# DanielPS555/Radix-sort-Merge-Sort-CUDA---Lab-y-practicos-GPGPU-2023

Hardware: AMD Instinct MI355X
Metric: Mkeys/s sorting uint32, n=2^28, 1 GPU (+ merge-sort at 2/4/8) (higher is better)
Workload: dtype u32; 1 GPU; LSD radix sort (8-bit digits, onesweep), n=2^28 uint32 u32, device-resident (BASELINE config 3); n_per_gpu=268435456, algo=radix, key=u32, dist=u32, parallelism=single GPU

## Files before the change

radix-sort-merge-sort-cuda---lab-y-practicos-gpgpu-2023_amd/csrc/segsort.hip:

```cpp
#include "segsort.h"

#include <algorithm>

#include "devutil.h"
#include "host.h"
#include "seg_kernels.h"

namespace labsort {

namespace {

constexpr int BIN_BLOCK = 1024, BIN_SPT = 4;

__global__ __launch_bounds__(BIN_BLOCK) void k_seg_bin(const uint32_t *__restrict__ off, uint32_t nseg, uint32_t n,
                                                        uint32_t max_len, SegEdges e, uint32_t copy1,
                                                        uint32_t *__restrict__ hdr, uint32_t *__restrict__ lists,
                                                        size_t stride, const Plan *__restrict__ hyplan) {
    __shared__ uint32_t cnt[SEG_CLASSES], base[SEG_CLASSES];
    if (hyplan && hyplan->hybrid == 0u) return;
    const uint32_t tid = threadIdx.x, lane = tid & 63u;
    if (tid < (uint32_t)SEG_CLASSES) cnt[tid] = 0u;
    __syncthreads();
    uint32_t cls[BIN_SPT], pos[BIN_SPT];
    bool bad = false;
#pragma unroll
    for (int j = 0; j < BIN_SPT; ++j) {
        const uint32_t seg = blockIdx.x * (uint32_t)(BIN_BLOCK * BIN_SPT) + (uint32_t)j * BIN_BLOCK + tid;
        uint32_t c = SEG_CLASSES;
        if (seg < nseg) {
            const uint32_t a = off[seg], b = off[seg + 1];
            if (b < a || b > n) {
                bad = true;
            } else {
                const uint32_t len = b - a;
                if (max_len && len > max_len) bad = true;
                if (len > 1u || (len == 1u && copy1)) {
                    c = 0u;
#pragma unroll
                    for (int q = 0; q < SEG_CLASSES - 1; ++q) c += len > e.e[q] ? 1u : 0u;
                }
            }
            if (seg == 0u && a != 0u) bad = true;
            if (seg == nseg - 1u && b != n) bad = true;
        }
        cls[j] = c;
        pos[j] = 0u;
        if (lists) {
#pragma unroll
            for (uint32_t cc = 0; cc < (uint32_t)SEG_CLASSES; ++cc) {
                const uint64_t m = __ballot(c == cc);
                if (m == 0ull) continue;
                const uint32_t leader = (uint32_t)__ffsll((long long)m) - 1u;
                uint32_t wb = 0u;
                if (lane == leader) wb = atomicAdd(&cnt[cc], (uint32_t)__popcll(m));
                wb = __shfl(wb, (int)leader);
                if (c == cc) pos[j] = wb + mbcnt64(m);
            }
        }
    }
    if (bad) atomicOr(hdr, 1u);
    if (!lists) return;
    __syncthreads();
    if (tid < (uint32_t)SEG_CLASSES) base[tid] = cnt[tid] ? atomicAdd(hdr + SEG_HDR_CNT + tid, cnt[tid]) : 0u;
    __syncthreads();
#pragma unroll
    for (int j = 0; j < BIN_SPT; ++j) {
        const uint32_t seg = blockIdx.x * (uint32_t)(BIN_BLOCK * BIN_SPT) + (uint32_t)j * BIN_BLOCK + tid;
        if (cls[j] < (uint32_t)SEG_CLASSES) lists[(size_t)cls[j] * stride + base[cls[j]] + pos[j]] = seg;
    }
}

__global__ __launch_bounds__(256) void k_seg_ids(const uint32_t *__restrict__ off, uint32_t nseg, uint32_t n,
                                                 const uint32_t *__restrict__ idx, uint32_t *__restrict__ ids,
                                                 uint32_t *__restrict__ iota, const uint32_t *__restrict__ hdr) {
    if (ld_agent(hdr) != 0u) return;
    const size_t stride = (size_t)gridDim.x * blockDim.x;
    for (size_t i = (size_t)blockIdx.x * blockDim.x + threadIdx.x; i < n; i += stride) {
        if (iota) iota[i] = (uint32_t)i;
        if (!ids) continue;
        uint32_t p = idx ? idx[i] : (uint32_t)i;
        if (p >= n) p = n - 1u;
        uint32_t lo = 1u, hi = nseg;
        while (lo < hi) {
            const uint32_t mid = lo + (hi - lo) / 2u;
            if (off[mid] > p) hi = mid;
            else lo = mid + 1u;
        }
        ids[i] = lo - 1u;
    }
}

__global__ __launch_bounds__(256) void k_seg_gather(const uint32_t *__restrict__ src, const uint32_t *__restrict__ vsrc,
                                                    const uint32_t *__restrict__ perm, uint32_t *__restrict__ out,
                                                    uint32_t *__restrict__ vout, uint32_t n,
                                                    const uint32_t *__restrict__ hdr) {
    if (ld_agent(hdr) != 0u) return;
    const size_t stride = (size_t)gridDim.x * blockDim.x;
    for (size_t i = (size_t)blockIdx.x * blockDim.x + threadIdx.x; i < n; i += stride) {
        uint32_t p = perm ? perm[i] : (uint32_t)i;
        if (p >= n) p = n - 1u;
        out[i] = src[p];
        if (vsrc) vout[i] = vsrc[p];
    }
}

__global__ void k_seg_err_acc(uint32_t *hdr, uint32_t *inner) {
    if (threadIdx.x == 0 && blockIdx.x == 0) {
        if (*inner) hdr[SEG_HDR_DEVERR] = 1u;
        *inner = 0u;
    }
}

unsigned stream_blocks(size_t n) {
    size_t b = (n + 256 * 8 - 1) / (256 * 8);
    return (unsigned)(b < 1 ? 1 : b > 8192 ? 8192 : b);
}

hipError_t launch_seg_sort(int c, const uint32_t *in, uint32_t *out, const uint32_t *vin, uint32_t *vout,
                           const uint32_t *off, const uint32_t *hdr, const uint32_t *list, uint32_t flip,
                           hipStream_t s, const HySel &hy = HySel{}, bool f32 = false) {
    return f32 ? launch_seg_sort_f32(c, in, out, vin, vout, off, hdr, list, flip, s, hy)
               : launch_seg_sort_t<false>(c, in, out, vin, vout, off, hdr, list, flip, s, hy);
}

hipError_t launch_seg_ids(const uint32_t *off, size_t nseg, size_t n, const uint32_t *idx, uint32_t *ids,
                          uint32_t *iota, const uint32_t *hdr, hipStream_t s) {
    k_seg_ids<<<stream_blocks(n), 256, 0, s>>>(off, (uint32_t)nseg, (uint32_t)n, idx, ids, iota, hdr);
    return hipGetLastError();
}

hipError_t launch_seg_gather(const uint32_t *src, const uint32_t *vsrc, const uint32_t *perm, uint32_t *out,
                             uint32_t *vout, size_t n, const uint32_t *hdr, hipStream_t s) {
    k_seg_gather<<<stream_blocks(n), 256, 0, s>>>(src, vsrc, perm, out, vout, (uint32_t)n, hdr);
    return hipGetLastError();
}

hipError_t launch_seg_err_acc(uint32_t *hdr, uint32_t *inner_err, hipStream_t s) {
    k_seg_err_acc<<<1, 64, 0, s>>>(hdr, inner_err);
    return hipGetLastError();
}

}

hipError_t launch_seg_bin(const uint32_t *off, size_t nseg, size_t n, size_t max_len, bool pairs, bool copy1,
                          uint32_t *hdr, uint32_t *lists, size_t stride, hipStream_t s) {
    const unsigned g = (unsigned)((nseg + BIN_BLOCK * BIN_SPT - 1) / (BIN_BLOCK * BIN_SPT));
    (void)pairs;
    const SegEdges e{{(uint32_t)SEG_WAVE_KEYS, (uint32_t)SEG_WAVE2_KEYS, (uint32_t)SEG_WAVE3_KEYS, (uint32_t)SEG_BLOCK_KEYS}};
    k_seg_bin<<<g, BIN_BLOCK, 0, s>>>(off, (uint32_t)nseg, (uint32_t)n, (uint32_t)max_len, e, copy1 ? 1u : 0u, hdr, lists,
                                      stride, nullptr);
    return hipGetLastError();
}

hipError_t launch_seg_lds_classes(size_t max_len, bool pairs, const uint32_t *in, uint32_t *out, const uint32_t *vin,
                                  uint32_t *vout, const uint32_t *off, const uint32_t *hdr, const uint32_t *lists,
                                  size_t stride, uint32_t flip, bool f32, hipStream_t s) {
    size_t edges[SEG_CLASSES];
    labsort_segment_class_edges(pairs ? 1 : 0, edges, SEG_CLASSES);
    int ncls = 1;
    while (ncls < SEG_CLASSES && max_len > edges[ncls - 1]) ++ncls;
    for (int c = 0; c < ncls; ++c) {
        const hipError_t e = launch_seg_sort(c, in, out, vin, vout, off, hdr, lists + (size_t)c * stride, flip, s, HySel{}, f32);
        if (e != hipSuccess) return e;
    }
    return hipSuccess;
}

namespace {
constexpr int FB_BLOCK = 1024;

__global__ __launch_bounds__(FB_BLOCK) void k_fin_bounds(const Plan *__restrict__ plan, Bufs bufs, uint32_t n, uint32_t flip,
                                                         const uint32_t *__restrict__ top14, uint32_t *__restrict__ off) {
    constexpr uint32_t GPB = FB_BLOCK / 4;
    __shared__ uint32_t wsum[FB_BLOCK / WAVE];
    __shared__ uint32_t gstart[GPB + 1];
    if (plan->hybrid == 0u) return;
    const uint32_t *__restrict__ keys = bufs.p[plan->fin_src];
    const uint32_t tid = threadIdx.x, lane = tid & 63u, wid = tid >> 6;
    const uint32_t g0 = blockIdx.x * GPB;
    uint32_t before = 0u;
    for (uint32_t i = tid; i < g0; i += FB_BLOCK) before += top14[i];
    const uint32_t mine = tid < GPB ? top14[g0 + tid] : 0u;
    uint32_t x = mine, tot = before;
#pragma unroll
    for (int o = 1; o < 64; o <<= 1) {
        const uint32_t t = __shfl_up(x, o);
        if (lane >= (uint32_t)o) x += t;
    }
#pragma unroll
    for (int o = 32; o > 0; o >>= 1) tot += __shfl_xor(tot, o);
    if (lane == 63u) wsum[wid] = x;
    __syncthreads();
    uint32_t pre = 0u;
    for (uint32_t w = 0; w < wid && w < GPB / WAVE; ++w) pre += wsum[w];
    __syncthreads();
    if (lane == 0u) wsum[wid] = tot;
    __syncthreads();
    uint32_t base = 0u;
    for (uint32_t w = 0; w < (uint32_t)(FB_BLOCK / WAVE); ++w) base += wsum[w];
    if (tid < GPB) {
        gstart[tid] = base + pre + x - mine;
        if (tid == GPB - 1u) gstart[GPB] = base + pre + x;
    }
    __syncthreads();
    const uint32_t q = blockIdx.x * FB_BLOCK + tid;
    uint32_t lo = min(gstart[tid >> 2], n), hi = min(gstart[(tid >> 2) + 1u], n);
    while (lo < hi) {
        const uint32_t mid = lo + (hi - lo) / 2u;
        if (((keys[mid] ^ flip) >> 16) >= q) hi = mid;
        else lo = mid + 1u;
    }
    off[q] = lo;
    if (q == HY_BUCKETS - 1u) off[HY_BUCKETS] = n;
}
}

hipError_t launch_hybrid_finish(const Plan *plan, Bufs b, size_t n, uint32_t flip, const uint32_t *top14, uint32_t *hdr,
                                uint32_t *off, uint32_t *lists, hipStream_t s) {
    static_assert(HY_BUCKETS % FB_BLOCK == 0 && HY_TOP * 4 == (int)HY_BUCKETS, "four buckets per top-14-bit group");
    const size_t stride = HY_BUCKETS;
    k_fin_bounds<<<HY_BUCKETS / FB_BLOCK, FB_BLOCK, 0, s>>>(plan, b, (uint32_t)n, flip, top14, off);
    hipError_t e = hipGetLastError();
    if (e != hipSuccess) return e;
    const SegEdges ed{{(uint32_t)SEG_WAVE_KEYS, (uint32_t)SEG_WAVE2_KEYS, (uint32_t)SEG_WAVE3_KEYS, (uint32_t)HY_BLOCK_KEYS}};
    k_seg_bin<<<HY_BUCKETS / (BIN_BLOCK * BIN_SPT), BIN_BLOCK, 0, s>>>(off, HY_BUCKETS, (uint32_t)n, HY_MAX_BUCKET, ed, 1u, hdr,
                                                                      lists, stride, plan);
    if ((e = hipGetLastError()) != hipSuccess) return e;
    const HySel hy{plan, {b.p[0], b.p[1], b.p[2]}};
    uint32_t *out = b.p[SEL_OUT];
    const unsigned cus = (unsigned)cu_count();
    for (int c = 0; c < SEG_CLASSES; ++c) {
        const uint32_t *list = lists + (size_t)c * stride;
        if (c == 3) {
            k_seg_block<HY_BLOCK, HY_BLOCK_KPT, false, HY_BLOCK_WPE><<<cus * (unsigned)HY_BLOCK_WPE, HY_BLOCK, 0, s>>>(
                out, out, nullptr, nullptr, off, hdr, list, 3, flip, hy);
            e = hipGetLastError();
        } else {
            e = launch_seg_sort(c, out, out, nullptr, nullptr, off, hdr, list, flip, s, hy);
        }
        if (e != hipSuccess) return e;
    }
    return hipSuccess;
}

size_t seg_inner_bytes(size_t n) {
    const size_t m = n < (size_t)LABSORT_AUTO_PAIRS_MERGE_MAX_KEYS ? n : (size_t)LABSORT_AUTO_PAIRS_MERGE_MAX_KEYS;
    return std::max(labsort_pairs_workspace_bytes(n, LABSORT_ALGO_AUTO), labsort_pairs_workspace_bytes(m, LABSORT_ALGO_MERGE));
}

}

using namespace labsort;

extern "C" {

size_t labsort_segment_tile_keys(void) { return (size_t)SEG_TILE_KEYS; }
size_t labsort_segment_pair_tile_keys(void) { return (size_t)SEG_TILE_PAIRS; }

int labsort_segment_class_edges(int pairs, size_t *edges, int cap) {
    const size_t e[SEG_CLASSES] = {(size_t)SEG_WAVE_KEYS, (size_t)SEG_WAVE2_KEYS, (size_t)SEG_WAVE3_KEYS, (size_t)SEG_BLOCK_KEYS,
                                   pairs ? (size_t)SEG_TILE_PAIRS : (size_t)SEG_TILE_KEYS};
    for (int i = 0; i < SEG_CLASSES && i < cap && edges; ++i) edges[i] = e[i];
    return SEG_CLASSES;
}

namespace {
bool seg_lds_path(size_t max_len, int pairs) {
    return max_len > 0 && max_len <= (pairs ? (size_t)SEG_TILE_PAIRS : (size_t)SEG_TILE_KEYS);
}
struct SegLayout {
    size_t off_lists, list_stride;
    size_t off_a, off_b, off_c, off_inner, inner_bytes;
    size_t total;
};
SegLayout seg_layout(size_t n, size_t nseg, bool lds) {
    SegLayout L{};
    Carver c{SEG_HDR_BYTES};
    if (lds) {
        L.list_stride = align_up(nseg * 4, 256) / 4;
        L.off_lists = c.take((size_t)SEG_CLASSES * L.list_stride * 4);
        L.total = c.o;
    } else {
        L.off_a = c.take(n * 4);
        L.off_b = c.take(n * 4);
        L.off_c = c.take(n * 4);
        L.off_inner = c.o;
        L.inner_bytes = seg_inner_bytes(n);
        L.total = c.o + L.inner_bytes;
    }
    return L;
}

int sort_segments(const uint32_t *ki, const uint32_t *vi, uint32_t *ko, uint32_t *vo, size_t n, const uint32_t *off,
                  size_t nseg, size_t max_len, int key_type, void *d_ws, size_t ws_bytes, void *stream) {
    const bool pairs = vi != nullptr || vo != nullptr;
    if (n == 0) return LABSORT_OK;
    if (!ki || !ko || !off || (pairs && (!vi || !vo))) return LABSORT_ERR_ARG;
    if (!device_key_type_ok(key_type)) return LABSORT_ERR_ARG;
    if (nseg == 0 || n > (size_t)0x7FFFFFFFu || nseg > (size_t)0x7FFFFFFFu) return LABSORT_ERR_ARG;
    if (pairs && !pairs_alias_ok(ki, vi, ko, vo)) return LABSORT_ERR_ARG;
    const bool lds = seg_lds_path(max_len, pairs ? 1 : 0);
    if (!lds && n > RADIX_MAX_N) return LABSORT_ERR_ARG;
    if (!d_ws || ws_bytes < labsort_segments_workspace_bytes(n, nseg, max_len, pairs ? 1 : 0)) return LABSORT_ERR_ARG;
    const SegLayout L = seg_layout(n, nseg, lds);
    const uint32_t flip = flip_of(key_type);
    hipStream_t s = as_stream(stream);
    char *ws = static_cast<char *>(d_ws);
    uint32_t *hdr = reinterpret_cast<uint32_t *>(ws);
    const bool inplace = ki == ko;
    HIP_TRY(launch_zero(hdr, SEG_HDR_BYTES, s));
    if (lds) {
        uint32_t *lists = reinterpret_cast<uint32_t *>(ws + L.off_lists);
        TimingScope ts(LABSORT_K_SEGSORT, s);
        HIP_TRY(launch_seg_bin(off, nseg, n, max_len, pairs, !inplace, hdr, lists, L.list_stride, s));
        HIP_TRY(launch_seg_lds_classes(max_len, pairs, ki, ko, vi, vo, off, hdr, lists, L.list_stride, flip,
                                       key_type == LABSORT_KEY_F32, s));
        return LABSORT_OK;
    }
    uint32_t *A = reinterpret_cast<uint32_t *>(ws + L.off_a), *B = reinterpret_cast<uint32_t *>(ws + L.off_b),
             *C = reinterpret_cast<uint32_t *>(ws + L.off_c);
    char *iws = ws + L.off_inner;
    uint32_t *ierr = reinterpret_cast<uint32_t *>(iws);
    HIP_TRY(launch_zero(ierr, 16, s));
    {
        TimingScope ts(LABSORT_K_SEGSORT, s);
        HIP_TRY(launch_seg_bin(off, nseg, n, max_len, pairs, false, hdr, nullptr, 0, s));
        if (pairs) HIP_TRY(launch_seg_ids(off, nseg, n, nullptr, nullptr, A, hdr, s));
        else HIP_TRY(launch_seg_ids(off, nseg, n, nullptr, A, nullptr, hdr, s));
    }
    int st;
    if ((st = labsort_sort_pairs_device(ki, A, B, C, n, key_type, LABSORT_ALGO_AUTO, iws, L.inner_bytes, stream))) return st;
    HIP_TRY(launch_seg_err_acc(hdr, ierr, s));
    if (pairs) {
        {
            TimingScope ts(LABSORT_K_SEGSORT, s);
            HIP_TRY(launch_seg_ids(off, nseg, n, C, B, nullptr, hdr, s));
        }
        if ((st = labsort_sort_pairs_device(B, C, B, C, n, LABSORT_KEY_U32, LABSORT_ALGO_AUTO, iws, L.inner_bytes, stream)))
            return st;
        HIP_TRY(launch_seg_err_acc(hdr, ierr, s));
        TimingScope ts(LABSORT_K_SEGSORT, s);
        if (inplace) {
            HIP_TRY(launch_seg_gather(ki, vi, C, A, B, n, hdr, s));
            HIP_TRY(launch_seg_gather(A, B, nullptr, ko, vo, n, hdr, s));
        } else {
            HIP_TRY(launch_seg_gather(ki, vi, C, ko, vo, n, hdr, s));
        }
    } else {
        if ((st = labsort_sort_pairs_device(C, B, C, B, n, LABSORT_KEY_U32, LABSORT_ALGO_AUTO, iws, L.inner_bytes, stream)))
            return st;
        HIP_TRY(launch_seg_err_acc(hdr, ierr, s));
        TimingScope ts(LABSORT_K_SEGSORT, s);
        HIP_TRY(launch_seg_gather(B, nullptr, nullptr, ko, nullptr, n, hdr, s));
    }
    return LABSORT_OK;
}
}

size_t labsort_segments_workspace_bytes(size_t n, size_t nseg, size_t max_segment_keys, int pairs) {
    return seg_layout(n, nseg, seg_lds_path(max_segment_keys, pairs)).total;
}

int labsort_sort_segments_device(const void *d_keys_in, void *d_keys_out, size_t n, const uint32_t *d_offsets,
                                 size_t nseg, size_t max_segment_keys, int key_type, void *d_ws, size_t ws_bytes,
                                 void *stream) {
    return sort_segments(static_cast<const uint32_t *>(d_keys_in), nullptr, static_cast<uint32_t *>(d_keys_out), nullptr,
                         n, d_offsets, nseg, max_segment_keys, key_type, d_ws, ws_bytes, stream);
}

int labsort_sort_segments_pairs_device(const void *d_keys_in, const void *d_vals_in, void *d_keys_out, void *d_vals_out,
                                       size_t n, const uint32_t *d_offsets, size_t nseg, size_t max_segment_keys,
                                       int key_type, void *d_ws, size_t ws_bytes, void *stream) {
    if (n == 0) return LABSORT_OK;
    if (!d_vals_in || !d_vals_out) return LABSORT_ERR_ARG;
    return sort_segments(static_cast<const uint32_t *>(d_keys_in), static_cast<const uint32_t *>(d_vals_in),
                         static_cast<uint32_t *>(d_keys_out), static_cast<uint32_t *>(d_vals_out), n, d_offsets, nseg,
                         max_segment_keys, key_type, d_ws, ws_bytes, stream);
}

int labsort_segments_workspace_status(const void *d_ws, void *stream) {
    uint32_t w[2] = {0, 0};
    if (const int st = read_ws_words(d_ws, w, 2, as_stream(stream))) return st;
    return w[0] ? LABSORT_ERR_ARG : w[SEG_HDR_DEVERR] ? LABSORT_ERR_DEVICE : LABSORT_OK;
}

}
```

Baseline: 135,100 Mkeys/s.

## Add dedicated finish kernel for large hybrid buckets with segment prefetch

Replaces the generic segmented block sort used for the largest bucket class in the hybrid radix finish with a specialized kernel. The new kernel runs two 8-bit LDS ranking passes over the low 16 bits, uses a DPP wave scan for the per-wave digit offsets, and prefetches the next segment's keys into registers while the current one is ranked and written. It also drops the flip/key-transform and extra buffer parameters. Register pressure rises from holding two key tiles, which may hurt occupancy. An A/B harness script for timing the finish stage is added.

```diff
diff --git a/harness/finish_ab.py b/harness/finish_ab.py
--- /dev/null
+++ b/harness/finish_ab.py
@@ -0,0 +1,97 @@
+#!/usr/bin/env python3
+import argparse
+import ctypes
+import importlib
+import os
+import statistics
+import sys
+
+import torch
+
+REPO = os.path.dirname(os.path.dirname(os.path.abspath(__file__)))
+sys.path.insert(0, REPO)
+ls = importlib.import_module("radix-sort-merge-sort-cuda---lab-y-practicos-gpgpu-2023_amd")
+
+K_SEGSORT = ls.KCLASS["segsort"]
+ALGO_RADIX = ls.ALGO["radix"]
+
+
+def load(path):
+    if not path:
+        return ls.lib
+    lib = ctypes.CDLL(path)
+    for name in ("labsort_sort_device", "labsort_workspace_bytes", "labsort_workspace_status", "labsort_radix_path",
+                 "labsort_timing_enable", "labsort_timing_read"):
+        f, g = getattr(lib, name), getattr(ls.lib, name)
+        f.argtypes, f.restype = g.argtypes, g.restype
+    return lib
+
+
+def fmt(ts):
+    return f"{statistics.median(ts):7.4f} [{min(ts):7.4f}, {max(ts):7.4f}]"
+
+
+def main():
+    ap = argparse.ArgumentParser()
+    ap.add_argument("--lib", action="append", default=[], help="NAME=PATH; empty PATH: the package's library")
+    ap.add_argument("--sizes", default="1,0.5,1.19", help="comma-separated, in units of 2^28 keys")
+    ap.add_argument("--reps", type=int, default=9)
+    ap.add_argument("--warmup", type=int, default=2)
+    ap.add_argument("--note", default="")
+    ap.add_argument("--out", default="")
+    a = ap.parse_args()
+    if not torch.cuda.is_available():
+        sys.exit("finish_ab: no GPU (no CPU fallback)")
+    out = open(a.out, "a") if a.out else sys.stdout
+    builds = {}
+    for spec in a.lib or ["this="]:
+        name, _, path = spec.partition("=")
+        builds[name] = load(path)
+    st = torch.cuda.current_stream().cuda_stream
+    print(f"# finish A/B{': ' + a.note if a.note else ''}: {torch.cuda.get_device_name(0)}; {a.reps} alternating repetitions "
+          f"after {a.warmup} warm-ups; ms per sort, median [min, max]", file=out)
+    for size in [float(x) for x in a.sizes.split(",")]:
+        n = int(size * (1 << 28))
+        if size == 1.0:
+            os.environ.pop("LABSORT_RADIX_HYBRID", None)
+        else:
+            os.environ["LABSORT_RADIX_HYBRID"] = "2"
+        keys = torch.empty(n, dtype=torch.int32, device="cuda")
+        ls.fill(keys, n, seed=0x5EED0001, dist="u32")
+        res = torch.empty_like(keys)
+        first = None
+        nbytes = max(int(lib.labsort_workspace_bytes(n, ALGO_RADIX)) for lib in builds.values())
+        ws = torch.zeros(nbytes, dtype=torch.uint8, device="cuda")
+        fin = {k: [] for k in builds}
+        tot = {k: [] for k in builds}
+        for rep in range(a.warmup + a.reps):
+            for name, lib in builds.items():
+                lib.labsort_timing_enable(1)
+                e0, e1 = torch.cuda.Event(enable_timing=True), torch.cuda.Event(enable_timing=True)
+                e0.record()
+                rc = lib.labsort_sort_device(keys.data_ptr(), res.data_ptr(), n, 0, ALGO_RADIX, ws.data_ptr(), nbytes, st)
+                e1.record()
+                e1.synchronize()
+                if rc or lib.labsort_workspace_status(ws.data_ptr(), n, ALGO_RADIX, st):
+                    sys.exit(f"finish_ab: {name}: the sort failed")
+                ms, cnt = ctypes.c_double(0.0), ctypes.c_longlong(0)
+                lib.labsort_timing_read(K_SEGSORT, ctypes.byref(ms), ctypes.byref(cnt))
+                lib.labsort_timing_enable(0)
+                if rep == 0:
+                    if int(lib.labsort_radix_path(ws.data_ptr(), n, st)) != 1:
+                        sys.exit(f"finish_ab: {name}: n = {n} did not take the hybrid path")
+                    if first is None:
+                        first = res.clone()
+                    elif not torch.equal(res, first):
+                        sys.exit(f"finish_ab: {name}: result differs from the first build's")
+                if rep >= a.warmup:
+                    fin[name].append(ms.value)
+                    tot[name].append(e0.elapsed_time(e1))
+        for name in builds:
+            print(f"n = {size:g} x 2^28  {name:>8}  finish {fmt(fin[name])}   whole sort (timing hooks on) {fmt(tot[name])}", file=out)
+        out.flush()
+        del keys, res, ws, first
+
+
+if __name__ == "__main__":
+    main()
diff --git a/radix-sort-merge-sort-cuda---lab-y-practicos-gpgpu-2023_amd/csrc/fin_block.h b/radix-sort-merge-sort-cuda---lab-y-practicos-gpgpu-2023_amd/csrc/fin_block.h
--- /dev/null
+++ b/radix-sort-merge-sort-cuda---lab-y-practicos-gpgpu-2023_amd/csrc/fin_block.h
@@ -0,0 +1,204 @@
+#pragma once
+#include "segsort.h"
+
+#include "devutil.h"
+
+namespace labsort {
+
+namespace {
+
+#ifndef LABSORT_FIN_PREFETCH
+#define LABSORT_FIN_PREFETCH 1
+#endif
+
+__device__ __forceinline__ uint32_t wave_incl_scan_dpp(uint32_t x) {
+    x += (uint32_t)__builtin_amdgcn_update_dpp(0, (int)x, 0x111, 0xf, 0xf, false);
+    x += (uint32_t)__builtin_amdgcn_update_dpp(0, (int)x, 0x112, 0xf, 0xf, false);
+    x += (uint32_t)__builtin_amdgcn_update_dpp(0, (int)x, 0x114, 0xf, 0xf, false);
+    x += (uint32_t)__builtin_amdgcn_update_dpp(0, (int)x, 0x118, 0xf, 0xf, false);
+    x += (uint32_t)__builtin_amdgcn_update_dpp(0, (int)x, 0x142, 0xa, 0xf, false);
+    x += (uint32_t)__builtin_amdgcn_update_dpp(0, (int)x, 0x143, 0xc, 0xf, false);
+    return x;
+}
+
+template <int BLOCK, int KPT>
+struct FinSmem {
+    static constexpr int R = 256, W = BLOCK / WAVE, TILE = BLOCK * KPT;
+    static_assert(TILE <= 65536, "16-bit LDS slots");
+    static_assert(W == 4, "the fold holds one counter row per wave in registers");
+    uint32_t keys[TILE];
+    alignas(16) uint32_t cnt[W * R];
+    alignas(16) uint32_t offs[W * R];
+    uint32_t probe[WAVE];
+    uint32_t ordered;
+};
+
+struct FinStripe {
+    size_t sb;
+    uint32_t ws0;
+    uint32_t nf;
+    uint32_t ng;
+    bool tail_ok;
+};
+template <int W, int KPT>
+__device__ __forceinline__ FinStripe fin_stripe(uint32_t b, uint32_t len, uint32_t lane, uint32_t wid) {
+    if (len > (uint32_t)(W * WAVE * KPT)) len = 0u;
+    const uint32_t jn = (len + (uint32_t)(W * WAVE) - 1u) / (uint32_t)(W * WAVE);
+    const uint32_t ws0 = wid * jn * WAVE;
+    const uint32_t rem = ws0 < len ? len - ws0 : 0u;
+    const uint32_t nf = min(jn, rem / WAVE);
+    const uint32_t tail = nf < jn ? rem - nf * WAVE : 0u;
+    return {(size_t)b + ws0, ws0, nf, nf + (tail ? 1u : 0u), lane < tail};
+}
+
+template <int KPT>
+__device__ __forceinline__ void fin_load(const uint32_t *in, const FinStripe &g, uint32_t lane, uint32_t (&k)[KPT]) {
+    const char *pb = reinterpret_cast<const char *>(in + g.sb);
+    const uint32_t lb = lane * 4u;
+    if (g.nf == (uint32_t)KPT) {
+#pragma unroll
+        for (int j = 0; j < KPT; ++j) k[j] = ld_stream<NT_TILE>(reinterpret_cast<const uint32_t *>(pb + (lb + (uint32_t)(j * WAVE * 4))));
+    } else {
+#pragma unroll
+        for (int j = 0; j < KPT; ++j) {
+            k[j] = 0xFFFFFFFFu;
+            if ((uint32_t)j < g.nf || ((uint32_t)j == g.nf && g.tail_ok))
+                k[j] = ld_stream<NT_TILE>(reinterpret_cast<const uint32_t *>(pb + (lb + (uint32_t)(j * WAVE * 4))));
+        }
+    }
+}
+
+template <int BLOCK, int KPT>
+__device__ __forceinline__ void fin_pass(FinSmem<BLOCK, KPT> &sm, const uint32_t (&k)[KPT], uint32_t shift, uint32_t ng,
+                                         bool atomic_rank, uint32_t lane, uint32_t wid) {
+    constexpr int W = FinSmem<BLOCK, KPT>::W, R = FinSmem<BLOCK, KPT>::R;
+    uint32_t *wh = sm.cnt + wid * R;
+    uint32_t *wo = sm.offs + wid * R;
+    uint32_t n0 = ng, n1 = ng;
+    asm volatile("" : "+s"(n0), "+s"(n1));
+    uint32_t z = 0u;
+    asm volatile("" : "+v"(z));
+    *reinterpret_cast<uint4 *>(wh + 4u * lane) = make_uint4(z, z, z, z);
+    uint32_t rank[KPT / 2] = {};
+#pragma unroll
+    for (int j = 0; j < KPT; ++j) {
+        uint32_t r = 0u;
+        if ((uint32_t)j < n0) r = rank8(wh, (k[j] >> shift) & 0xFFu, lane, atomic_rank);
+        set16(rank, j, r);
+    }
+    __syncthreads();
+    {
+        uint4 c[W];
+#pragma unroll
+        for (int w = 0; w < W; ++w) c[w] = *reinterpret_cast<const uint4 *>(sm.cnt + w * R + 4u * lane);
+        uint32_t tot[4] = {0u, 0u, 0u, 0u}, bef[4] = {0u, 0u, 0u, 0u};
+#pragma unroll
+        for (int w = 0; w < W; ++w) {
+            const uint32_t cw[4] = {c[w].x, c[w].y, c[w].z, c[w].w};
+            const bool before = (uint32_t)w < wid;
+#pragma unroll
+            for (int q = 0; q < 4; ++q) {
+                tot[q] += cw[q];
+                bef[q] += before ? cw[q] : 0u;
+            }
+        }
+        const uint32_t s = tot[0] + tot[1] + tot[2] + tot[3];
+        uint32_t run = wave_incl_scan_dpp(s) - s;
+        uint4 o4;
+        o4.x = run + bef[0];
+        run += tot[0];
+        o4.y = run + bef[1];
+        run += tot[1];
+        o4.z = run + bef[2];
+        run += tot[2];
+        o4.w = run + bef[3];
+        *reinterpret_cast<uint4 *>(wo + 4u * lane) = o4;
+    }
+    __builtin_amdgcn_wave_barrier();
+#pragma unroll
+    for (int j = 0; j < KPT; ++j)
+        if ((uint32_t)j < n1) set16(rank, j, wo[(k[j] >> shift) & 0xFFu] + get16(rank, j));
+#pragma unroll
+    for (int j = 0; j < KPT; ++j)
+        if ((uint32_t)j < n1) sm.keys[get16(rank, j)] = k[j];
+    __syncthreads();
+}
+
+template <int BLOCK, int KPT, int WPE>
+__global__ __launch_bounds__(BLOCK, WPE) void k_fin_block(uint32_t *out, const uint32_t *__restrict__ off,
+                                                           const uint32_t *__restrict__ hdr,
+                                                           const uint32_t *__restrict__ list, HySel hy) {
+    using S = FinSmem<BLOCK, KPT>;
+    constexpr int W = S::W;
+    constexpr int CLS = 3;
+    constexpr bool PREFETCH = LABSORT_FIN_PREFETCH != 0;
+    __shared__ S sm;
+    if (hy.plan->hybrid == 0u) return;
+    const uint32_t *in = hy.buf[hy.plan->fin_src];
+    if (ld_agent(hdr) != 0u) return;
+    const uint32_t cnt = hdr[SEG_HDR_CNT + CLS];
+    const uint32_t tid = threadIdx.x, lane = tid & 63u, wid = __builtin_amdgcn_readfirstlane(tid >> 6);
+    if (blockIdx.x >= cnt) return;
+    probe_lane_order(sm.probe, &sm.ordered, lane, wid);
+    __syncthreads();
+    const bool atomic_rank = lane_order_probed(&sm.ordered);
+    uint32_t nb, ne;
+    {
+        const uint32_t seg = __builtin_amdgcn_readfirstlane(list[blockIdx.x]);
+        nb = __builtin_amdgcn_readfirstlane(off[seg]);
+        ne = __builtin_amdgcn_readfirstlane(off[seg + 1]);
+    }
+    uint32_t k[KPT];
+    FinStripe g = fin_stripe<W, KPT>(nb, ne - nb, lane, wid);
+    if constexpr (PREFETCH) fin_load(in, g, lane, k);
+    for (uint32_t it = blockIdx.x; it < cnt; it += gridDim.x) {
+        if constexpr (!PREFETCH) {
+            g = fin_stripe<W, KPT>(nb, ne - nb, lane, wid);
+            fin_load(in, g, lane, k);
+        }
+        const bool more = it + gridDim.x < cnt;
+        if (more) {
+            const uint32_t seg = __builtin_amdgcn_readfirstlane(list[it + gridDim.x]);
+            nb = __builtin_amdgcn_readfirstlane(off[seg]);
+            ne = __builtin_amdgcn_readfirstlane(off[seg + 1]);
+        }
+        fin_pass(sm, k, 0u, g.ng, atomic_rank, lane, wid);
+        {
+            uint32_t n2 = g.ng;
+            asm volatile("" : "+s"(n2));
+#pragma unroll
+            for (int j = 0; j < KPT; ++j)
+                if ((uint32_t)j < n2) k[j] = sm.keys[g.ws0 + (uint32_t)j * WAVE + lane];
+        }
+        fin_pass(sm, k, 8u, g.ng, atomic_rank, lane, wid);
+        FinStripe gn = g;
+        uint32_t kn[PREFETCH ? KPT : 1];
+        if constexpr (PREFETCH) {
+            gn = fin_stripe<W, KPT>(nb, more ? ne - nb : 0u, lane, wid);
+            fin_load(in, gn, lane, kn);
+        }
+        uint32_t nfs = g.nf;
+        asm volatile("" : "+s"(nfs));
+        const uint32_t *sk = sm.keys + g.ws0 + lane;
+        char *ob = reinterpret_cast<char *>(out + g.sb);
+        const uint32_t lb = lane * 4u;
+        if (nfs == (uint32_t)KPT) {
+#pragma unroll
+            for (int j = 0; j < KPT; ++j) *reinterpret_cast<uint32_t *>(ob + (lb + (uint32_t)(j * WAVE * 4))) = sk[j * WAVE];
+        } else {
+#pragma unroll
+            for (int j = 0; j < KPT; ++j)
+                if ((uint32_t)j < nfs || ((uint32_t)j == nfs && g.tail_ok))
+                    *reinterpret_cast<uint32_t *>(ob + (lb + (uint32_t)(j * WAVE * 4))) = sk[j * WAVE];
+        }
+        if constexpr (PREFETCH) {
+            g = gn;
+#pragma unroll
+            for (int j = 0; j < KPT; ++j) k[j] = kn[j];
+        }
+    }
+}
+
+}
+
+}
diff --git a/radix-sort-merge-sort-cuda---lab-y-practicos-gpgpu-2023_amd/csrc/segsort.hip b/radix-sort-merge-sort-cuda---lab-y-practicos-gpgpu-2023_amd/csrc/segsort.hip
--- a/radix-sort-merge-sort-cuda---lab-y-practicos-gpgpu-2023_amd/csrc/segsort.hip
+++ b/radix-sort-merge-sort-cuda---lab-y-practicos-gpgpu-2023_amd/csrc/segsort.hip
@@ -3,6 +3,7 @@
 #include <algorithm>
 
 #include "devutil.h"
+#include "fin_block.h"
 #include "host.h"
 #include "seg_kernels.h"
 
@@ -232,8 +233,7 @@
     for (int c = 0; c < SEG_CLASSES; ++c) {
         const uint32_t *list = lists + (size_t)c * stride;
         if (c == 3) {
-            k_seg_block<HY_BLOCK, HY_BLOCK_KPT, false, HY_BLOCK_WPE><<<cus * (unsigned)HY_BLOCK_WPE, HY_BLOCK, 0, s>>>(
-                out, out, nullptr, nullptr, off, hdr, list, 3, flip, hy);
+            k_fin_block<HY_BLOCK, HY_BLOCK_KPT, HY_BLOCK_WPE><<<cus * (unsigned)HY_BLOCK_WPE, HY_BLOCK, 0, s>>>(out, off, hdr, list, hy);
             e = hipGetLastError();
         } else {
             e = launch_seg_sort(c, out, out, nullptr, nullptr, off, hdr, list, flip, s, hy);
```

After: 142,100 Mkeys/s, median of 6. +5.2%, better.
